# yuxng/PoseCNN

Measured on AMD Instinct MI355X. Metric: RGB-D frames/sec (640x480, 21 classes), higher is better.
Workload: dtype f32

## Files before the change

posecnn_amd/csrc/mfma_ring.h:

```cpp
#pragma once

namespace pcnn {

typedef float v4f __attribute__((ext_vector_type(4)));

__device__ __forceinline__ void glds16_s(const char* sbase, unsigned voff, unsigned lds_addr)
{
  asm volatile("s_mov_b32 m0, %2\n\tglobal_load_lds_dwordx4 %0, %1"
               :: "v"(voff), "s"(sbase), "s"(lds_addr) : "memory", "m0");
}

__device__ __forceinline__ int ring_src_col(int lr, int row) { return (lr ^ (row & 15)) * 4; }
__device__ __forceinline__ unsigned ring_chunk_bytes(int j, int lk, int lr) { return (unsigned)(((4 * j + lk) ^ lr) * 16); }

}

#define RING_DSREAD_B128(DST, ADDR, OFF) asm volatile("ds_read_b128 %0, %1 offset:%2" : "=v"(DST) : "v"(ADDR), "i"(OFF))

#define RING_GLOAD_B128(DST, SBASE, VOFF, OFF) \
  asm volatile("global_load_dwordx4 %0, %1, %2 offset:%3" : "=v"(DST) : "v"(VOFF), "s"(SBASE), "i"(OFF) : "memory")
```

posecnn_amd/csrc/wino_mfma.hip:

```cpp
#include <cstdlib>

#include "pcnn_device.h"
#include "mfma_ring.h"
#include "../../include/posecnn_hip_wino_packed.h"

namespace {

using namespace pcnn;

constexpr int WM_BC = 64;
constexpr int WM_KC = 64;
constexpr int WM_LD = 64;
constexpr int WM_NBUF = 3;
constexpr int WM_BT = 32;
constexpr int WM_NW = 4;
constexpr int WM_UB = WM_BC / 4 / WM_NW;

enum : int {
  ABL_NO_BARRIER = 1,
  ABL_NO_DMA = 2,
  ABL_NO_LDS_READS = 4,
  ABL_NO_MFMA = 8,
  ABL_NO_FOLD = 16,
  ABL_NO_EPILOGUE = 32,
  ABL_L2_OPERANDS = 64,
  ABL_NO_STORES = 128,
  ABL_EPI_REGS_ONLY = 256,
  ABL_NT_STORES = 512,
  ABL_NO_B_LOADS = 1024,
};

template <int POOL, int BSRC = 0, int ABL = 0, int ODD = 0>
__global__ __launch_bounds__(64 * WM_NW, 2) void wino43_mfma_kernel(
    const float* __restrict__ v, const float* __restrict__ ut, const float* __restrict__ bias,
    float* __restrict__ y, float* __restrict__ ypool, int H, int W, int Cin, int Cout, int Ht, int Wt,
    long long T, long long tiles_per_group, int relu, int nbt, int ncb, int ksplit, long long ysplit_stride, int mode)
{
  constexpr int RING = WM_NBUF * (WM_BT + (BSRC == 0 ? 64 : 0)) * WM_LD, STAGE2 = 2 * WM_BT * 4 * 64;
  __shared__ __attribute__((aligned(16))) float smem[RING > STAGE2 ? RING : STAGE2];

  const int x = blockIdx.x & 7, q = blockIdx.x >> 3;
  const bool cbmajor = (mode & 1) != 0;
  const int cb = cbmajor ? x : q % ncb;
  const int tb = cbmajor ? q : (q / ncb) * 8 + x;
  if (tb >= nbt) return;
  const int tb_data = (ABL & ABL_L2_OPERANDS) ? 0 : tb, cb_data = (ABL & ABL_L2_OPERANDS) ? 0 : cb;
  y += (long long)blockIdx.y * ysplit_stride;

  const int tid = threadIdx.x, lane = tid & 63;
  const int wave = __builtin_amdgcn_readfirstlane(tid >> 6);
  const int lr = lane & 15, lk = lane >> 4;
  const int nbg = (int)((tiles_per_group + WM_BT - 1) / WM_BT);
  const int grp = tb / nbg;
  const long long t0 = (long long)grp * tiles_per_group + (long long)(tb_data - (ABL & ABL_L2_OPERANDS ? 0 : grp * nbg)) * WM_BT;
  const long long tend = (long long)(grp + 1) * tiles_per_group;
  const float* utg = ut + (size_t)grp * 36 * Cout * Cin;
  const int ks = blockIdx.y;
  const int NK = Cin / WM_KC / ksplit;

  const int dr0 = 8 * wave + lk, dr1 = dr0 + 4;
  const int dc0 = ring_src_col(lr, dr0), dc1 = ring_src_col(lr, dr1);
  const int ur0 = 4 * WM_UB * wave + lk;
  const long long tlast = tend - 1;
  const long long ta0 = t0 + dr0 < tend ? t0 + dr0 : tlast, ta1 = t0 + dr1 < tend ? t0 + dr1 : tlast;
  const unsigned va0 = (unsigned)((ta0 * Cin + dc0) * 4), va1 = (unsigned)((ta1 * Cin + dc1) * 4);
  unsigned ub[WM_UB];
#pragma unroll
  for (int i = 0; i < WM_UB; i++) ub[i] = (unsigned)((((size_t)(cb_data * WM_BC + ur0 + 4 * i)) * Cin + ring_src_col(lr, ur0 + 4 * i)) * 4);
  const char* vbase = reinterpret_cast<const char*>(v);
  const char* ubase = reinterpret_cast<const char*>(utg);
  const long long vplane = T * Cin;
  const long long uplane = (long long)Cout * Cin;
  const int ldsw = 8 * wave * WM_LD;
  const int ldsu = 4 * WM_UB * wave * WM_LD;
  const unsigned lds_base_ = (unsigned)(unsigned long long)(__attribute__((address_space(3))) float*)smem;
  const unsigned lds_a0 = lds_base_ + (unsigned)ldsw * 4u;
  const unsigned lds_b0 = lds_base_ + (unsigned)(WM_NBUF * WM_BT * WM_LD + ldsu) * 4u;

  const float bv = bias ? bias[(size_t)grp * Cout + cb * WM_BC + 16 * wave + lr] : 0.f;
  v4f acc[6][2];
#pragma unroll
  for (int i = 0; i < 6; i++) acc[i][0] = acc[i][1] = (v4f){0.f, 0.f, 0.f, 0.f};
  typedef float v2f __attribute__((ext_vector_type(2)));
  v2f yo2[2][2][16];
#define YO(B_, I_, O_) yo2[B_][(I_) >> 1][O_][(I_) & 1]
#pragma unroll
  for (int b = 0; b < 2; b++)
#pragma unroll
    for (int i = 0; i < 2; i++)
#pragma unroll
      for (int o = 0; o < 16; o++) yo2[b][i][o] = (v2f){0.f, 0.f};

#define WM_DMA(BUF, VO, UO)                                                  \
  if constexpr (!(ABL & ABL_NO_DMA)) {                                       \
    const char* vs_ = vbase + (VO) * 4;                                      \
    const char* us_ = ubase + (UO) * 4;                                      \
    const unsigned la_ = lds_a0 + (unsigned)(BUF) * (WM_BT * WM_LD * 4);       \
    const unsigned lb_ = lds_b0 + (unsigned)(BUF) * (64 * WM_LD * 4);          \
    glds16_s(vs_, va0, la_);                                                 \
    glds16_s(vs_, va1, la_ + 4 * WM_LD * 4);                                 \
    if constexpr (BSRC == 0) {                                               \
      _Pragma("unroll") for (int i_ = 0; i_ < WM_UB; i_++)                    \
        glds16_s(us_, ub[i_], lb_ + 4 * i_ * WM_LD * 4);                      \
    }                                                                        \
  }

  int pnu = 0, pxi = 0, pkc = 0;
  constexpr int WM_USTEP = BSRC == 0 ? WM_KC : 16 * WM_KC;
  long long pvo = (long long)ks * NK * WM_KC;
  long long puo = BSRC == 0 ? pvo : ((long long)(cb_data * (WM_BC / 16) + wave) * (Cin / WM_KC) + (long long)ks * NK) * WM_USTEP;
  const long long kback = (long long)(NK - 1) * WM_KC, ukback = (long long)(NK - 1) * WM_USTEP;
  const long long dvx = 6 * vplane - kback, dux = 6 * uplane - ukback;
  const long long dvn = -29 * vplane - kback, dun = -29 * uplane - ukback;
#define WM_PF_ADVANCE()                                                                          \
  do {                                                                                           \
    if (pkc + 1 < NK) { pkc++; pvo += WM_KC; puo += WM_USTEP; }                 \
    else if (pxi < 5) { pkc = 0; pxi++; pvo += dvx; puo += dux; }        \
    else if (pnu < 5) { pkc = 0; pxi = 0; pnu++; pvo += dvn; puo += dun; }        \
  } while (0)
  v4f bq[4][2];
  if constexpr (BSRC == 1 && (ABL & ABL_NO_B_LOADS)) {
#pragma unroll
    for (int i = 0; i < 4; i++) bq[i][0] = bq[i][1] = (v4f){1.f, 1.f, 1.f, 1.f};
  }
  const unsigned vbo = 16u * (unsigned)lane;
  long long pub = 0;
#define WM_BLOAD(S, UO, J0)                                                  \
  if constexpr (!(ABL & ABL_NO_B_LOADS)) {                                   \
    const char* us_ = ubase + (UO) * 4;                                      \
    RING_GLOAD_B128(S[0], us_, vbo, (J0) * 1024);                            \
    RING_GLOAD_B128(S[1], us_, vbo, (J0) * 1024 + 1024);                     \
  }
  if constexpr (BSRC == 0) {
    { WM_DMA(0, pvo, puo); WM_PF_ADVANCE(); }
    { WM_DMA(1, pvo, puo); WM_PF_ADVANCE(); }
  } else {
    WM_BLOAD(bq[0], puo, 0);
    WM_BLOAD(bq[1], puo, 2);
    { WM_DMA(0, pvo, puo); WM_PF_ADVANCE(); }
    { WM_DMA(1, pvo, puo); pub = puo; WM_PF_ADVANCE(); }
  }
  int cur = 0;

  const int ra0 = lr * WM_LD, rb = (16 * wave + lr) * WM_LD;

  v4f xa0[2], xa1[2], xb[2], ya0[2], ya1[2], yb[2];
  const unsigned lds0 = (unsigned)(unsigned long long)(__attribute__((address_space(3))) float*)smem;
  unsigned adA[4], adB[4];
#pragma unroll
  for (int j = 0; j < 4; j++) {
    const unsigned chb = ring_chunk_bytes(j, lk, lr);
    adA[j] = lds0 + (unsigned)ra0 * 4u + chb;
    adB[j] = lds0 + (unsigned)(WM_NBUF * WM_BT * WM_LD + rb) * 4u + chb;
  }
#define WM_DSREAD(DST, ADDR, OFF)                                                                     \
  if constexpr (!(ABL & ABL_NO_LDS_READS)) RING_DSREAD_B128(DST, ADDR, OFF);                          \
  else asm volatile("" : "+v"(DST) : "v"(ADDR))
#define WM_READ_AT(SA0, SA1, SB, G0, CUR)                                                             \
  _Pragma("unroll") for (int g_ = 0; g_ < 2; g_++) {                                                  \
    WM_DSREAD(SB[g_], adB[(G0) + g_], (CUR) * (64 * WM_LD * 4));                                      \
    WM_DSREAD(SA0[g_], adA[(G0) + g_], (CUR) * (WM_BT * WM_LD * 4));                                  \
    WM_DSREAD(SA1[g_], adA[(G0) + g_], (CUR) * (WM_BT * WM_LD * 4) + 4096);       \
  }
#define WM_READ(SA0, SA1, SB, G0)                                                                     \
  if constexpr (ABL & ABL_NO_LDS_READS) { WM_READ_AT(SA0, SA1, SB, G0, 0); }    \
  else if (cur == 0) { WM_READ_AT(SA0, SA1, SB, G0, 0); }                                             \
  else if (cur == 1) { WM_READ_AT(SA0, SA1, SB, G0, 1); }                                             \
  else { WM_READ_AT(SA0, SA1, SB, G0, 2); }
#define WM_READA_AT(SA0, SA1, G0, CUR)                                                                \
  _Pragma("unroll") for (int g_ = 0; g_ < 2; g_++) {                                                  \
    WM_DSREAD(SA0[g_], adA[(G0) + g_], (CUR) * (WM_BT * WM_LD * 4));                                  \
    WM_DSREAD(SA1[g_], adA[(G0) + g_], (CUR) * (WM_BT * WM_LD * 4) + 4096);                           \
  }
#define WM_READA(SA0, SA1, G0)                                                                        \
  if constexpr (ABL & ABL_NO_LDS_READS) { WM_READA_AT(SA0, SA1, G0, 0); }                             \
  else if (cur == 0) { WM_READA_AT(SA0, SA1, G0, 0); }                                                \
  else if (cur == 1) { WM_READA_AT(SA0, SA1, G0, 1); }                                                \
  else { WM_READA_AT(SA0, SA1, G0, 2); }
  static_assert(WM_NBUF == 3, "WM_READ dispatches over a ring of three buffers");
#define WM_MFMA1(SA0, SA1, SB, G, ACC)                                                                \
  if constexpr (ABL & ABL_NO_MFMA) { asm volatile("" :: "v"(SA0[G]), "v"(SA1[G]), "v"(SB[G])); } else \
  _Pragma("unroll") for (int i_ = 0; i_ < 4; i_++) {                                                  \
    ACC[0] = __builtin_amdgcn_mfma_f32_16x16x4f32(SA0[G][i_], SB[G][i_], ACC[0], 0, 0, 0);            \
    ACC[1] = __builtin_amdgcn_mfma_f32_16x16x4f32(SA1[G][i_], SB[G][i_], ACC[1], 0, 0, 0);            \
  }
#define WM_MFMA(SA0, SA1, SB, ACC)                                                                    \
  WM_MFMA1(SA0, SA1, SB, 0, ACC) WM_MFMA1(SA0, SA1, SB, 1, ACC)
#define WM_MFMA1_Z(SA0, SA1, SB, G, ACC)                                                              \
  if constexpr (ABL & ABL_NO_MFMA) { asm volatile("" :: "v"(SA0[G]), "v"(SA1[G]), "v"(SB[G])); } else { \
    const v4f z_ = (v4f){0.f, 0.f, 0.f, 0.f};                                                         \
    ACC[0] = __builtin_amdgcn_mfma_f32_16x16x4f32(SA0[G][0], SB[G][0], z_, 0, 0, 0);                  \
    ACC[1] = __builtin_amdgcn_mfma_f32_16x16x4f32(SA1[G][0], SB[G][0], z_, 0, 0, 0);                  \
    _Pragma("unroll") for (int i_ = 1; i_ < 4; i_++) {                                                \
      ACC[0] = __builtin_amdgcn_mfma_f32_16x16x4f32(SA0[G][i_], SB[G][i_], ACC[0], 0, 0, 0);          \
      ACC[1] = __builtin_amdgcn_mfma_f32_16x16x4f32(SA1[G][i_], SB[G][i_], ACC[1], 0, 0, 0);          \
    }                                                                                                 \
  }
#define WM_FOLD(NU)                                                                                   \
  if constexpr (!(ABL & ABL_NO_FOLD)) {                                                               \
    const int n_ = (NU);                                                                              \
    const float c0 = n_ == 5 ? 0.f : 1.f;                                                             \
    const float c1 = n_ == 1 ? 1.f : n_ == 2 ? -1.f : n_ == 3 ? 2.f : n_ == 4 ? -2.f : 0.f;           \
    const float c2 = (n_ == 1 || n_ == 2) ? 1.f : (n_ == 3 || n_ == 4) ? 4.f : 0.f;                   \
    const float c3 = n_ == 1 ? 1.f : n_ == 2 ? -1.f : n_ == 3 ? 8.f : n_ == 4 ? -8.f : n_ == 5 ? 1.f : 0.f; \
     \
     \
     \
     \
     \
    _Pragma("unroll") for (int b_ = 0; b_ < 2; b_++)                                                \
      _Pragma("unroll") for (int h_ = 0; h_ < 2; h_++) {                                            \
        v2f m_[6], t_[4];                                                                           \
        _Pragma("unroll") for (int x_ = 0; x_ < 6; x_++) m_[x_] = (v2f){acc[x_][b_][2 * h_], acc[x_][b_][2 * h_ + 1]}; \
        const v2f s_ = m_[1] + m_[2], d_ = m_[1] - m_[2], S_ = m_[3] + m_[4], D_ = m_[3] - m_[4];   \
        t_[0] = (m_[0] + s_) + S_;                                                                  \
        t_[1] = __builtin_elementwise_fma((v2f){2.f, 2.f}, D_, d_);                                 \
        t_[2] = __builtin_elementwise_fma((v2f){4.f, 4.f}, S_, s_);                                 \
        t_[3] = __builtin_elementwise_fma((v2f){8.f, 8.f}, D_, d_) + m_[5];                         \
        _Pragma("unroll") for (int a_ = 0; a_ < 4; a_++) {                                          \
          yo2[b_][h_][4 * a_ + 0] = __builtin_elementwise_fma(t_[a_], (v2f){c0, c0}, yo2[b_][h_][4 * a_ + 0]); \
          yo2[b_][h_][4 * a_ + 1] = __builtin_elementwise_fma(t_[a_], (v2f){c1, c1}, yo2[b_][h_][4 * a_ + 1]); \
          yo2[b_][h_][4 * a_ + 2] = __builtin_elementwise_fma(t_[a_], (v2f){c2, c2}, yo2[b_][h_][4 * a_ + 2]); \
          yo2[b_][h_][4 * a_ + 3] = __builtin_elementwise_fma(t_[a_], (v2f){c3, c3}, yo2[b_][h_][4 * a_ + 3]); \
        }                                                                                           \
      }                                                                                             \
  }

#define WM_STAGE0(XI, XP)                                                                             \
  do {                                                                                                \
    if constexpr (ABL & ABL_NO_BARRIER) asm volatile("s_waitcnt vmcnt(4) lgkmcnt(0)" ::: "memory");   \
    else asm volatile("s_waitcnt vmcnt(6) lgkmcnt(0)\n\ts_barrier" ::: "memory");                     \
    WM_READ(xa0, xa1, xb, 0);                                                                         \
    __builtin_amdgcn_sched_barrier(0);    \
    if (kc > 0) { WM_MFMA(ya0, ya1, yb, acc[XI]); }                                                   \
    else if ((XI) > 0) { WM_MFMA(ya0, ya1, yb, acc[XP]); }                                            \
    else if (nu > 0) { WM_MFMA(ya0, ya1, yb, acc[5]); WM_FOLD(nup); }                                 \
    {                                                                                                 \
      const int nb = cur >= 1 ? cur - 1 : 2;            \
      WM_DMA(nb, pvo, puo);                                                                           \
      WM_PF_ADVANCE();                                                                                \
    }                                                                                                 \
    __builtin_amdgcn_sched_barrier(0);                                                                \
    asm volatile("s_waitcnt lgkmcnt(0)" ::: "memory");           \
    __builtin_amdgcn_sched_barrier(0);                                                                \
    if (kc == 0) { WM_MFMA1_Z(xa0, xa1, xb, 0, acc[XI]); }           \
    else { WM_MFMA1(xa0, xa1, xb, 0, acc[XI]); }                                                      \
    __builtin_amdgcn_sched_barrier(0);    \
    WM_READ(ya0, ya1, yb, 2);                                                                         \
    __builtin_amdgcn_sched_barrier(0);                                                                \
    WM_MFMA1(xa0, xa1, xb, 1, acc[XI]);                                                               \
    __builtin_amdgcn_sched_barrier(0);                                                                \
    asm volatile("s_waitcnt lgkmcnt(0)" ::: "memory");    \
    cur = cur == 2 ? 0 : cur + 1;                                                                     \
  } while (0)
  static_assert(2 + WM_UB == 6, "the stage barrier's vmcnt(6) counts the 2 + WM_UB DMA instructions a wave issues per stage");

  constexpr int WM_VM1 = WM_BT / 4 / WM_NW;
#define WM_YMFMA_R(SB, ACC)                                                                           \
  __builtin_amdgcn_sched_barrier(0); WM_MFMA(ya0, ya1, SB, ACC); __builtin_amdgcn_sched_barrier(0)
#define WM_STAGE1(XI, XP, P, KC)                                                                      \
  do {                                                                                                \
    if constexpr (ABL & ABL_NO_BARRIER) asm volatile("s_waitcnt vmcnt(2) lgkmcnt(0)" ::: "memory");   \
    else asm volatile("s_waitcnt vmcnt(2) lgkmcnt(0)\n\ts_barrier" ::: "memory");                     \
    WM_READA(xa0, xa1, 0);                                                                            \
    WM_BLOAD(bq[2 - 2 * (P)], pub, 0);                     \
    __builtin_amdgcn_sched_barrier(0);                                                                \
    if ((KC) > 0) { WM_YMFMA_R(bq[3 - 2 * (P)], acc[XI]); }                                           \
    else if ((XI) > 0) { WM_YMFMA_R(bq[3 - 2 * (P)], acc[XP]); }                                      \
    else if (nu > 0) { WM_YMFMA_R(bq[3 - 2 * (P)], acc[5]); WM_FOLD(nup); }                           \
    __builtin_amdgcn_sched_barrier(0);                                                                \
               \
    WM_BLOAD(bq[3 - 2 * (P)], pub, 2);                                                                \
    {                                                                                                 \
      const int nb = cur >= 1 ? cur - 1 : 2;            \
      WM_DMA(nb, pvo, puo);                                                                           \
      pub = puo;                                                                                      \
      WM_PF_ADVANCE();                                                                                \
    }                                                                                                 \
    __builtin_amdgcn_sched_barrier(0);                                                                \
    asm volatile("s_waitcnt lgkmcnt(0)" ::: "memory");           \
    __builtin_amdgcn_sched_barrier(0);                                                                \
    if ((KC) == 0) { WM_MFMA1_Z(xa0, xa1, bq[2 * (P)], 0, acc[XI]); }    \
    else { WM_MFMA1(xa0, xa1, bq[2 * (P)], 0, acc[XI]); }                                             \
    __builtin_amdgcn_sched_barrier(0);                                                                \
    WM_READA(ya0, ya1, 2);                                                                            \
    __builtin_amdgcn_sched_barrier(0);                                                                \
    WM_MFMA1(xa0, xa1, bq[2 * (P)], 1, acc[XI]);                                                      \
    __builtin_amdgcn_sched_barrier(0);                                                                \
    asm volatile("s_waitcnt lgkmcnt(0)" ::: "memory");                                                \
    cur = cur == 2 ? 0 : cur + 1;                                                                     \
  } while (0)
  static_assert(WM_VM1 == 2, "the stage barrier's vmcnt(2) of BSRC = 1 counts the A DMA instructions a wave issues per stage");
#define WM_PLANE_E(XI, XP) for (int kc = 0; kc < NK; kc += 2) { WM_STAGE1(XI, XP, 0, kc); WM_STAGE1(XI, XP, 1, kc + 1); }
#define WM_PLANE_O(XI, XP, P0)                                                                        \
  WM_STAGE1(XI, XP, P0, 0);                                                                           \
  for (int kc = 1; kc < NK; kc += 2) { WM_STAGE1(XI, XP, 1 - (P0), kc); WM_STAGE1(XI, XP, P0, kc + 1); }

  int nup = -1;
  if constexpr (BSRC == 0) {
    for (int nu = 0; nu < 6; nu++) {
      for (int kc = 0; kc < NK; kc++) WM_STAGE0(0, 5);
      for (int kc = 0; kc < NK; kc++) WM_STAGE0(1, 0);
      for (int kc = 0; kc < NK; kc++) WM_STAGE0(2, 1);
      for (int kc = 0; kc < NK; kc++) WM_STAGE0(3, 2);
      for (int kc = 0; kc < NK; kc++) WM_STAGE0(4, 3);
      for (int kc = 0; kc < NK; kc++) WM_STAGE0(5, 4);
      nup = nu;
    }
  } else if constexpr (ODD == 0) {
    for (int nu = 0; nu < 6; nu++) {
      WM_PLANE_E(0, 5) WM_PLANE_E(1, 0) WM_PLANE_E(2, 1) WM_PLANE_E(3, 2) WM_PLANE_E(4, 3) WM_PLANE_E(5, 4)
      nup = nu;
    }
  } else {
    for (int nu = 0; nu < 6; nu++) {
      WM_PLANE_O(0, 5, 0) WM_PLANE_O(1, 0, 1) WM_PLANE_O(2, 1, 0) WM_PLANE_O(3, 2, 1) WM_PLANE_O(4, 3, 0) WM_PLANE_O(5, 4, 1)
      nup = nu;
    }
  }
  if constexpr (BSRC == 0) {
    asm volatile("s_waitcnt lgkmcnt(0)" ::: "memory");
    __builtin_amdgcn_sched_barrier(0);
    WM_MFMA(ya0, ya1, yb, acc[5]);
  } else {
    asm volatile("s_waitcnt vmcnt(2) lgkmcnt(0)" ::: "memory");
    __builtin_amdgcn_sched_barrier(0);
    WM_MFMA(ya0, ya1, bq[3], acc[5]);
  }
  WM_FOLD(5);
  asm volatile("s_waitcnt vmcnt(0)" ::: "memory");
  __syncthreads();
#undef WM_STAGE0
#undef WM_STAGE1
#undef WM_YMFMA_R
#undef WM_PLANE_E
#undef WM_PLANE_O
#undef WM_BLOAD
#undef WM_READA
#undef WM_READA_AT
#undef WM_READ
#undef WM_READ_AT
#undef WM_DSREAD
#undef WM_MFMA
#undef WM_MFMA1
#undef WM_MFMA1_Z
#undef WM_FOLD
#undef WM_DMA
#undef WM_PF_ADVANCE

  if constexpr (ABL & ABL_EPI_REGS_ONLY) {
    const float bv_ = bv;
    float k_ = 0.f;
#pragma unroll
    for (int b = 0; b < 2; b++)
#pragma unroll
      for (int i = 0; i < 4; i++)
#pragma unroll
        for (int o = 0; o < 16; o++) { float val = YO(b, i, o) + bv_; if (relu) val = val > 0.f ? val : 0.f; k_ += val; }
    if (k_ == 12345.678f) y[tid] = k_;
    return;
  }
  if constexpr (ABL & ABL_NO_EPILOGUE) {
    float k_ = 0.f;
#pragma unroll
    for (int b = 0; b < 2; b++)
#pragma unroll
      for (int i = 0; i < 4; i++)
#pragma unroll
        for (int o = 0; o < 16; o++) k_ += YO(b, i, o);
#pragma unroll
    for (int x_ = 0; x_ < 6; x_++) k_ += acc[x_][0][0] + acc[x_][1][1];
    if (k_ == 12345.678f) y[tid] = k_;
    return;
  }
  const int col = 16 * wave + lr;
#pragma unroll
  for (int b = 0; b < 2; b++)
#pragma unroll
    for (int i = 0; i < 4; i++)
#pragma unroll
      for (int o = 0; o < 16; o++) {
        float val = YO(b, i, o) + bv;
        if (relu) val = val > 0.f ? val : 0.f;
        YO(b, i, o) = val;
      }

  constexpr int SYF = WM_BT * 4 * 64;
  const int wcol = col ^ (16 * lk);
  const int HtWt = Ht * Wt;
  const int bimg0 = (int)(t0 / HtWt);
  const int rem0 = (int)(t0 - (long long)bimg0 * HtWt);
  const int ty0 = rem0 / Wt, tx0 = rem0 - ty0 * Wt;
  const int re = (tid >> 4) & 3, rc4 = (tid & 15) * 4;
  int s_img[8], s_tyx[8];
#pragma unroll
  for (int r = 0; r < 8; r++) {
    const int tl = wave + WM_NW * r;
    const unsigned n = (unsigned)(tx0 + tl), q = n / (unsigned)Wt, tx = n - q * (unsigned)Wt;
    const unsigned m = (unsigned)ty0 + q, q2 = m / (unsigned)Ht, ty = m - q2 * (unsigned)Ht;
    s_img[r] = bimg0 + (int)q2;
    s_tyx[r] = t0 + tl < tend ? (int)(ty | (tx << 16)) : 0xffff;
  }
  if (POOL != 1) {
#pragma unroll
    for (int a = 0; a < 4; a++) {
      float* sY = smem + (a & 1) * SYF;
#pragma unroll
      for (int b = 0; b < 2; b++)
#pragma unroll
        for (int i = 0; i < 4; i++) {
          const int tl = 16 * b + 4 * lk + i;
#pragma unroll
          for (int e = 0; e < 4; e++) sY[(tl * 4 + e) * 64 + wcol] = YO(b, i, 4 * a + e);
        }
      __syncthreads();
#pragma unroll
      for (int r = 0; r < 8; r++) {
        const int tl = wave + WM_NW * r;
        const int ty = s_tyx[r] & 0xffff, tx = s_tyx[r] >> 16;
        const int oy = 4 * ty + a, ox = 4 * tx + re;
        if (oy < H && ox < W) {
          const v4f o4 = *reinterpret_cast<const v4f*>(&sY[(tl * 4 + re) * 64 + (rc4 ^ (16 * ((tl >> 2) & 3)))]);
          if constexpr (ABL & ABL_NO_STORES) { if (o4[0] == 12345.678f) y[tid] = o4[1]; }
          else if constexpr (ABL & ABL_NT_STORES) __builtin_nontemporal_store(o4, reinterpret_cast<v4f*>(y + (((long long)s_img[r] * H + oy) * W + ox) * Cout + cb * WM_BC + rc4));
          else *reinterpret_cast<v4f*>(y + (((long long)s_img[r] * H + oy) * W + ox) * Cout + cb * WM_BC + rc4) = o4;
        }
      }
    }
  }
  if (POOL != 0) {
    float* yp = POOL == 1 ? y : ypool;
    float* sY = smem;
    const int Hp = H / 2, Wp = W / 2;
#pragma unroll
    for (int b = 0; b < 2; b++)
#pragma unroll
      for (int i = 0; i < 4; i++) {
        const int tl = 16 * b + 4 * lk + i;
#pragma unroll
        for (int a2 = 0; a2 < 2; a2++)
#pragma unroll
          for (int e2 = 0; e2 < 2; e2++) {
            float p = YO(b, i, 4 * (2 * a2) + 2 * e2);
            const float p1 = YO(b, i, 4 * (2 * a2) + 2 * e2 + 1), p2 = YO(b, i, 4 * (2 * a2 + 1) + 2 * e2),
                        p3 = YO(b, i, 4 * (2 * a2 + 1) + 2 * e2 + 1);
            p = p1 > p ? p1 : p;
            p = p2 > p ? p2 : p;
            p = p3 > p ? p3 : p;
            sY[(tl * 4 + 2 * a2 + e2) * 64 + wcol] = p;
          }
      }
    __syncthreads();
#pragma unroll
    for (int r = 0; r < 8; r++) {
      const int tl = wave + WM_NW * r;
      const int ty = s_tyx[r] & 0xffff, tx = s_tyx[r] >> 16;
      const int py = 2 * ty + (re >> 1), px = 2 * tx + (re & 1);
      if (py < Hp && px < Wp)
        *reinterpret_cast<v4f*>(yp + (((long long)s_img[r] * Hp + py) * Wp + px) * Cout + cb * WM_BC + rc4) =
            *reinterpret_cast<const v4f*>(&sY[(tl * 4 + re) * 64 + (rc4 ^ (16 * ((tl >> 2) & 3)))]);
    }
  }
}

#undef YO

template <int POOL>
__global__ __launch_bounds__(256) void wino43_splitk_reduce_kernel(
    const float* __restrict__ part, int S, long long stride, const float* __restrict__ bias, int relu,
    float* __restrict__ y, float* __restrict__ ypool, int B, int H, int W, int C, int imgs_per_group)
{
  const int c4n = C >> 2;
  const int Ho = POOL ? H / 2 : H, Wo = POOL ? W / 2 : W;
  const long long total = (long long)B * Ho * Wo * c4n;
  for (long long i = (long long)blockIdx.x * 256 + threadIdx.x; i < total; i += (long long)gridDim.x * 256) {
    const int c4 = (int)(i % c4n) * 4;
    long long r = i / c4n;
    const int ox = (int)(r % Wo); r /= Wo;
    const int oy = (int)(r % Ho);
    const int b = (int)(r / Ho);
    const v4f bv = *reinterpret_cast<const v4f*>(bias + (size_t)(b / imgs_per_group) * C + c4);
    v4f best = (v4f){0.f, 0.f, 0.f, 0.f};
#pragma unroll
    for (int q = 0; q < (POOL ? 4 : 1); q++) {
      const int yy = POOL ? 2 * oy + (q >> 1) : oy, xx = POOL ? 2 * ox + (q & 1) : ox;
      const long long o = (((long long)b * H + yy) * W + xx) * C + c4;
      v4f v = *reinterpret_cast<const v4f*>(part + o);
      for (int s2 = 1; s2 < S; s2++) v += *reinterpret_cast<const v4f*>(part + s2 * stride + o);
      v += bv;
      if (relu) {
#pragma unroll
        for (int e = 0; e < 4; e++) v[e] = v[e] > 0.f ? v[e] : 0.f;
      }
      if (POOL != 1) *reinterpret_cast<v4f*>(y + o) = v;
      if (q == 0) best = v;
      else {
#pragma unroll
        for (int e = 0; e < 4; e++) best[e] = v[e] > best[e] ? v[e] : best[e];
      }
    }
    if (POOL != 0) {
      float* yp = POOL == 1 ? y : ypool;
      *reinterpret_cast<v4f*>(yp + (((long long)b * Ho + oy) * Wo + ox) * C + c4) = best;
    }
  }
}

int wino43_cin_split(long long nbt, int ncb, int Cin)
{
  const int NK = Cin / WM_KC;
  int S = 1;
  if (nbt * ncb >= 128) return 1;
  while (S < 8 && nbt * ncb * S * 2 <= 512 && NK % (2 * S) == 0) S *= 2;
  return S;
}

}

extern "C" int pcnn_winograd43_conv_workspace_bytes(int B, int H, int W, int Cin, int Cout, int groups, size_t* bytes)
{
  PCNN_REQUIRE(bytes, PCNN_ENULL, "winograd43_conv_workspace_bytes: NULL output");
  PCNN_REQUIRE(B >= 1 && H >= 1 && W >= 1 && Cin >= 64 && Cout >= 64 && groups >= 1 && B % groups == 0, PCNN_EINVAL,
               "winograd43_conv_workspace_bytes: bad shape");
  const long long tpg = (long long)B * ((H + 3) / 4) * ((W + 3) / 4) / groups;
  const int S = wino43_cin_split((long long)groups * ((tpg + WM_BT - 1) / WM_BT), Cout / WM_BC, Cin);
  *bytes = S > 1 ? sizeof(float) * ((size_t)S * B * H * W * Cout + (size_t)groups * Cout) : 0;
  return PCNN_OK;
}

static int wino43_conv_launch(bool packed, const float* v, const float* ut, const float* bias, int B, int H,
                              int W, int Cin, int Cout, int groups, int relu, int pool,
                              float* y, float* y_pool, void* workspace, size_t workspace_bytes,
                              void* stream_)
{
  PCNN_REQUIRE(B >= 1 && H >= 1 && W >= 1, PCNN_EINVAL, "winograd43_conv: bad shape %dx%dx%d", B, H, W);
  PCNN_REQUIRE(Cin >= 64 && Cin % 64 == 0, PCNN_EINVAL, "winograd43_conv: input channels must be a multiple of 64 (got %d)", Cin);
  PCNN_REQUIRE(Cout >= 64 && Cout % 64 == 0, PCNN_EINVAL, "winograd43_conv: output channels must be a multiple of 64 (got %d)", Cout);
  PCNN_REQUIRE(pool >= 0 && pool <= 2, PCNN_EINVAL, "winograd43_conv: pool must be 0 (none), 1 (pooled only) or 2 (both)");
  PCNN_REQUIRE(!pool || (H % 2 == 0 && W % 2 == 0), PCNN_EINVAL, "winograd43_conv: pooling needs even height/width");
  PCNN_REQUIRE(groups >= 1 && B % groups == 0, PCNN_EINVAL, "winograd43_conv: batch %d is not a multiple of groups %d", B, groups);
  PCNN_REQUIRE(v && ut && bias && y && (pool != 2 || y_pool), PCNN_ENULL, "winograd43_conv: NULL pointer");
  PCNN_REQUIRE(aligned16(v) && aligned16(ut) && aligned16(bias) && aligned16(y) && (pool != 2 || aligned16(y_pool)), PCNN_EINVAL,
               "winograd43_conv: pointers (v, ut, bias, y, y_pool) must be 16-byte aligned");
  hipStream_t stream = (hipStream_t)stream_;
  const int Ht = (H + 3) / 4, Wt = (W + 3) / 4;
  const long long T = (long long)B * Ht * Wt;
  const long long tpg = T / groups;
  const int ncb = Cout / WM_BC;
  const long long nbt = (long long)groups * ((tpg + WM_BT - 1) / WM_BT);
  const long long blocks = ((nbt + 7) / 8) * 8 * ncb;
  PCNN_REQUIRE(blocks < (1ll << 31), PCNN_EINVAL, "winograd43_conv: grid too large");
  PCNN_REQUIRE(T * Cin < (1ll << 30) && (long long)Cout * Cin < (1ll << 30), PCNN_EINVAL,
               "winograd43_conv: a transform plane of %lld x %d (or %d x %d) floats exceeds the kernel's 32-bit byte offsets", T, Cin, Cout, Cin);
  int S = wino43_cin_split(nbt, ncb, Cin);
  const size_t out_elems = (size_t)B * H * W * Cout;
  if (S > 1 && !(workspace && aligned16(workspace) && workspace_bytes >= sizeof(float) * (S * out_elems + (size_t)groups * Cout))) S = 1;
  static const int env_mode = [] { const char* e = getenv("PCNN_WINO_MODE"); return e ? atoi(e) : -1; }();
  const double u_bytes = 36.0 * Cout * (double)Cin * 4.0 * groups, v_bytes = 36.0 * (double)T * Cin * 4.0;
  int mode = (ncb == 8 && u_bytes > v_bytes) ? 1 : 0;
  if (env_mode >= 0) mode = ((env_mode & 1) && ncb == 8) ? 1 : 0;
  const long long nblocks = (mode & 1) ? 8 * nbt : blocks;
#define WM_GO_(K, Y, BIAS, RELU, KS, STRIDE) PCNN_LAUNCH(K, dim3((unsigned)nblocks, KS), dim3(64 * WM_NW), 0, stream, v, ut, BIAS, Y, y_pool, \
                             H, W, Cin, Cout, Ht, Wt, T, tpg, RELU, (int)nbt, ncb, KS, (long long)(STRIDE), mode)
#define WM_GO(P, Y, BIAS, RELU, KS, STRIDE)                                      \
  do {                                                                           \
    if (packed && ((Cin / WM_KC / (KS)) & 1)) WM_GO_((wino43_mfma_kernel<P, 1, 0, 1>), Y, BIAS, RELU, KS, STRIDE); \
    else if (packed) WM_GO_((wino43_mfma_kernel<P, 1>), Y, BIAS, RELU, KS, STRIDE);   \
    else WM_GO_((wino43_mfma_kernel<P>), Y, BIAS, RELU, KS, STRIDE);             \
  } while (0)
  if (S == 1) {
    if (pool == 0) WM_GO(0, y, bias, relu, 1, 0); else if (pool == 1) WM_GO(1, y, bias, relu, 1, 0); else WM_GO(2, y, bias, relu, 1, 0);
  } else {
    float* part = static_cast<float*>(workspace);
    WM_GO(0, part, (const float*)nullptr, 0, S, out_elems);
    const long long items = (long long)B * (pool ? (H / 2) * (W / 2) : H * W) * (Cout / 4);
    const unsigned rgrid = (unsigned)((items + 255) / 256 < 65536 ? (items + 255) / 256 : 65536);
    if (pool == 0)
      PCNN_LAUNCH(wino43_splitk_reduce_kernel<0>, dim3(rgrid), dim3(256), 0, stream, part, S, (long long)out_elems, bias, relu, y, y_pool, B, H, W, Cout, B / groups);
    else if (pool == 1)
      PCNN_LAUNCH(wino43_splitk_reduce_kernel<1>, dim3(rgrid), dim3(256), 0, stream, part, S, (long long)out_elems, bias, relu, y, y_pool, B, H, W, Cout, B / groups);
    else
      PCNN_LAUNCH(wino43_splitk_reduce_kernel<2>, dim3(rgrid), dim3(256), 0, stream, part, S, (long long)out_elems, bias, relu, y, y_pool, B, H, W, Cout, B / groups);
  }
  return check_launch(packed ? "winograd43_conv_packed_fwd" : "winograd43_conv_fwd");
}

extern "C" int pcnn_winograd43_conv_fwd(const float* v, const float* ut, const float* bias, int B, int H,
                                        int W, int Cin, int Cout, int groups, int relu, int pool,
                                        float* y, float* y_pool, void* workspace, size_t workspace_bytes,
                                        void* stream_)
{
  return wino43_conv_launch(false, v, ut, bias, B, H, W, Cin, Cout, groups, relu, pool, y, y_pool, workspace, workspace_bytes, stream_);
}

extern "C" int pcnn_winograd43_conv_packed_fwd(const float* v, const float* utp, const float* bias, int B, int H,
                                               int W, int Cin, int Cout, int groups, int relu, int pool,
                                               float* y, float* y_pool, void* workspace, size_t workspace_bytes,
                                               void* stream_)
{
  return wino43_conv_launch(true, v, utp, bias, B, H, W, Cin, Cout, groups, relu, pool, y, y_pool, workspace, workspace_bytes, stream_);
}

namespace {

__global__ __launch_bounds__(256) void wino43_pack_filters_kernel(const float* __restrict__ ut, float* __restrict__ utp,
                                                                  int Cin, int Cout, long long total4)
{
  const int nkc = Cin / WM_KC, n16n = Cout / 16;
  for (long long o = (long long)blockIdx.x * 256 + threadIdx.x; o < total4; o += (long long)gridDim.x * 256) {
    const int l = (int)(o & 63), j = (int)((o >> 6) & 3);
    long long r = o >> 8;
    const int kc = (int)(r % nkc); r /= nkc;
    const int n16 = (int)(r % n16n);
    const long long gk = r / n16n;
    const int lr = l & 15, lk = l >> 4;
    const long long src = (gk * Cout + 16 * n16 + lr) * Cin + 64 * kc + 16 * j + 4 * lk;
    *reinterpret_cast<v4f*>(utp + 4 * o) = *reinterpret_cast<const v4f*>(ut + src);
  }
}

}

extern "C" int pcnn_winograd43_pack_filters_fwd(const float* ut, int Cin, int Cout, int groups, float* utp, void* stream_)
{
  PCNN_REQUIRE(Cin >= 64 && Cin % 64 == 0, PCNN_EINVAL, "winograd43_pack_filters: input channels must be a multiple of 64 (got %d)", Cin);
  PCNN_REQUIRE(Cout >= 64 && Cout % 64 == 0, PCNN_EINVAL, "winograd43_pack_filters: output channels must be a multiple of 64 (got %d)", Cout);
  PCNN_REQUIRE(groups >= 1, PCNN_EINVAL, "winograd43_pack_filters: groups must be positive (got %d)", groups);
  PCNN_REQUIRE(ut && utp, PCNN_ENULL, "winograd43_pack_filters: NULL pointer");
  PCNN_REQUIRE(ut != utp, PCNN_EINVAL, "winograd43_pack_filters: not an in-place permutation");
  PCNN_REQUIRE(aligned16(ut) && aligned16(utp), PCNN_EINVAL, "winograd43_pack_filters: pointers (ut, utp) must be 16-byte aligned");
  hipStream_t stream = (hipStream_t)stream_;
  const long long total4 = (long long)groups * 36 * Cout * Cin / 4;
  const unsigned grid = (unsigned)((total4 + 255) / 256 < 65536 ? (total4 + 255) / 256 : 65536);
  PCNN_LAUNCH(wino43_pack_filters_kernel, dim3(grid), dim3(256), 0, stream, ut, utp, Cin, Cout, total4);
  return check_launch("winograd43_pack_filters_fwd");
}
```

Before: 840.4.

## Restructure Winograd epilogue with scalar store bases and fused bias-relu per row

Measured after the change: 840.2. About the same (-0.0%).

```diff
diff --git a/posecnn_amd/csrc/mfma_ring.h b/posecnn_amd/csrc/mfma_ring.h
--- a/posecnn_amd/csrc/mfma_ring.h
+++ b/posecnn_amd/csrc/mfma_ring.h
@@ -19,3 +19,10 @@
 
 #define RING_GLOAD_B128(DST, SBASE, VOFF, OFF) \
   asm volatile("global_load_dwordx4 %0, %1, %2 offset:%3" : "=v"(DST) : "v"(VOFF), "s"(SBASE), "i"(OFF) : "memory")
+
+#define RING_GSTORE_B128(SBASE, VOFF, DATA, MOD)                                                      \
+  do {                                                                                                \
+    unsigned long long sb_;                                                                           \
+    asm volatile("s_mov_b64 %0, %3\n\tglobal_store_dwordx4 %1, %2, %0" MOD "\n\ts_nop 1"             \
+                 : "=&s"(sb_) : "v"(VOFF), "v"(DATA), "s"(SBASE) : "memory");                         \
+  } while (0)
diff --git a/posecnn_amd/csrc/wino_mfma.hip b/posecnn_amd/csrc/wino_mfma.hip
--- a/posecnn_amd/csrc/wino_mfma.hip
+++ b/posecnn_amd/csrc/wino_mfma.hip
@@ -373,70 +373,109 @@
     if (k_ == 12345.678f) y[tid] = k_;
     return;
   }
-  const int col = 16 * wave + lr;
-#pragma unroll
-  for (int b = 0; b < 2; b++)
-#pragma unroll
-    for (int i = 0; i < 4; i++)
-#pragma unroll
-      for (int o = 0; o < 16; o++) {
-        float val = YO(b, i, o) + bv;
-        if (relu) val = val > 0.f ? val : 0.f;
-        YO(b, i, o) = val;
-      }
+  const int elane = (int)__builtin_amdgcn_mbcnt_hi(~0u, __builtin_amdgcn_mbcnt_lo(~0u, 0u));
+  const int elr = elane & 15, elk = elane >> 4;
+  const int col = 16 * wave + elr;
+#define WM_BIAS_RELU(B0, B1, I0, I1, O0, O1)                                                           \
+  if (relu) {                                                                                          \
+    _Pragma("unroll") for (int b_ = (B0); b_ < (B1); b_++)                                             \
+      _Pragma("unroll") for (int i_ = (I0); i_ < (I1); i_++)                                           \
+        _Pragma("unroll") for (int o_ = (O0); o_ < (O1); o_++) {                                       \
+          const float val = YO(b_, i_, o_) + bv;                                                       \
+          YO(b_, i_, o_) = val > 0.f ? val : 0.f;                                                      \
+        }                                                                                              \
+  } else {                                                                                             \
+    _Pragma("unroll") for (int b_ = (B0); b_ < (B1); b_++)                                             \
+      _Pragma("unroll") for (int i_ = (I0); i_ < (I1); i_++)                                           \
+        _Pragma("unroll") for (int o_ = (O0); o_ < (O1); o_++) YO(b_, i_, o_) = YO(b_, i_, o_) + bv;   \
+  }
 
   constexpr int SYF = WM_BT * 4 * 64;
-  const int wcol = col ^ (16 * lk);
-  const int HtWt = Ht * Wt;
-  const int bimg0 = (int)(t0 / HtWt);
-  const int rem0 = (int)(t0 - (long long)bimg0 * HtWt);
-  const int ty0 = rem0 / Wt, tx0 = rem0 - ty0 * Wt;
-  const int re = (tid >> 4) & 3, rc4 = (tid & 15) * 4;
-  int s_img[8], s_tyx[8];
-#pragma unroll
-  for (int r = 0; r < 8; r++) {
-    const int tl = wave + WM_NW * r;
-    const unsigned n = (unsigned)(tx0 + tl), q = n / (unsigned)Wt, tx = n - q * (unsigned)Wt;
-    const unsigned m = (unsigned)ty0 + q, q2 = m / (unsigned)Ht, ty = m - q2 * (unsigned)Ht;
-    s_img[r] = bimg0 + (int)q2;
-    s_tyx[r] = t0 + tl < tend ? (int)(ty | (tx << 16)) : 0xffff;
-  }
+  const int wcol = col ^ (16 * elk);
+  const int re = elk, rc4 = elr * 4;
+#define WM_SLOT_COORDS(LANE)                                                                           \
+  const unsigned HtWt = (unsigned)Ht * (unsigned)Wt;                                                   \
+  const unsigned l_t = (unsigned)t0 + (unsigned)(wave + WM_NW * ((LANE) & 7));                         \
+  const unsigned l_img = l_t / HtWt, l_rem = l_t - l_img * HtWt;                                       \
+  const unsigned l_ty = l_rem / (unsigned)Wt, l_tx = l_rem - l_ty * (unsigned)Wt;                      \
+  const bool l_live = (long long)l_t < tend
+#define WM_SLOT32(V, R) __builtin_amdgcn_readlane((int)(V), R)
+#define WM_SLOT64(V, R) (((unsigned long long)(unsigned)__builtin_amdgcn_readlane((int)((unsigned long long)(V) >> 32), R) << 32) | \
+                         (unsigned)__builtin_amdgcn_readlane((int)(unsigned)(unsigned long long)(V), R))
+  typedef __attribute__((address_space(3))) const float* lds_cfp;
+  lds_cfp srd[4];
+#pragma unroll
+  for (int c = 0; c < 4; c++) srd[c] = (lds_cfp)smem + (wave * 4 + re) * 64 + (rc4 ^ (16 * c));
+#define WM_EPI_READ(O4, BUF)                                                                           \
+  _Pragma("unroll") for (int r = 0; r < 8; r++)                                                        \
+    O4[r] = *reinterpret_cast<__attribute__((address_space(3))) const v4f*>(srd[r & 3] + (BUF) * SYF + r * (WM_NW * 4 * 64)); \
+  asm volatile("" ::: "memory")
   if (POOL != 1) {
+    WM_SLOT_COORDS(elane);
+    const int l_rows = l_live ? min(H - 4 * (int)l_ty, 4) : 0, l_cols = min(W - 4 * (int)l_tx, 4);
+    const unsigned long long l_base = (unsigned long long)y + 4ull * (unsigned long long)((((long long)l_img * H + 4 * l_ty) * W + 4 * l_tx) * Cout + cb * WM_BC);
+    const int l_whole = l_cols == 4 ? l_rows : 0;
+    const long long pitch = 4ll * W * Cout;
+    const unsigned vst = (unsigned)(re * Cout + rc4) * 4u;
+    int s_rc[8];
+    unsigned long long s_base[8];
+#pragma unroll
+    for (int r = 0; r < 8; r++) { s_rc[r] = WM_SLOT32(l_rows | (l_cols << 4), r); s_base[r] = WM_SLOT64(l_base, r); }
 #pragma unroll
     for (int a = 0; a < 4; a++) {
       float* sY = smem + (a & 1) * SYF;
+      WM_BIAS_RELU(0, 2, 0, 4, 4 * a, 4 * a + 4);
 #pragma unroll
       for (int b = 0; b < 2; b++)
 #pragma unroll
         for (int i = 0; i < 4; i++) {
-          const int tl = 16 * b + 4 * lk + i;
+          const int tl = 16 * b + 4 * elk + i;
 #pragma unroll
           for (int e = 0; e < 4; e++) sY[(tl * 4 + e) * 64 + wcol] = YO(b, i, 4 * a + e);
         }
       __syncthreads();
-#pragma unroll
-      for (int r = 0; r < 8; r++) {
-        const int tl = wave + WM_NW * r;
-        const int ty = s_tyx[r] & 0xffff, tx = s_tyx[r] >> 16;
-        const int oy = 4 * ty + a, ox = 4 * tx + re;
-        if (oy < H && ox < W) {
-          const v4f o4 = *reinterpret_cast<const v4f*>(&sY[(tl * 4 + re) * 64 + (rc4 ^ (16 * ((tl >> 2) & 3)))]);
-          if constexpr (ABL & ABL_NO_STORES) { if (o4[0] == 12345.678f) y[tid] = o4[1]; }
-          else if constexpr (ABL & ABL_NT_STORES) __builtin_nontemporal_store(o4, reinterpret_cast<v4f*>(y + (((long long)s_img[r] * H + oy) * W + ox) * Cout + cb * WM_BC + rc4));
-          else *reinterpret_cast<v4f*>(y + (((long long)s_img[r] * H + oy) * W + ox) * Cout + cb * WM_BC + rc4) = o4;
+      v4f o4[8];
+      WM_EPI_READ(o4, a & 1);
+      const unsigned long long arow = (unsigned long long)(a * pitch);
+#define WM_EPI_STORE(R)                                                                                \
+      do {                                                                                             \
+        const char* dst = reinterpret_cast<const char*>(s_base[R] + arow);    \
+        if constexpr (ABL & ABL_NO_STORES) { if (o4[R][0] == 12345.678f) y[tid] = o4[R][1]; }          \
+        else if constexpr (ABL & ABL_NT_STORES) RING_GSTORE_B128(dst, vst, o4[R], " nt");              \
+        else RING_GSTORE_B128(dst, vst, o4[R], "");                                                    \
+      } while (0)
+      if ((__builtin_amdgcn_ballot_w64(a < l_whole) & 0xffull) == 0xffull) {
+#pragma unroll
+        for (int r = 0; r < 8; r++) WM_EPI_STORE(r);
+      } else {
+#pragma unroll
+        for (int r = 0; r < 8; r++) {
+          const int rows = s_rc[r] & 15, cols = s_rc[r] >> 4;
+          if (a < rows) {
+            if (cols == 4) WM_EPI_STORE(r);
+            else if (re < cols) WM_EPI_STORE(r);
+          }
         }
       }
+#undef WM_EPI_STORE
     }
   }
   if (POOL != 0) {
     float* yp = POOL == 1 ? y : ypool;
     float* sY = smem;
     const int Hp = H / 2, Wp = W / 2;
+    int plane = elane;
+    if (POOL == 2) asm volatile("" : "+v"(plane));
+    WM_SLOT_COORDS(plane);
+    const int l_rows = l_live ? min(Hp - 2 * (int)l_ty, 2) : 0, l_cols = min(Wp - 2 * (int)l_tx, 2);
+    const unsigned long long l_base = (unsigned long long)yp + 4ull * (unsigned long long)((((long long)l_img * Hp + 2 * l_ty) * Wp + 2 * l_tx) * Cout + cb * WM_BC);
+    const unsigned vst = (unsigned)(((re >> 1) * Wp + (re & 1)) * Cout + rc4) * 4u;
 #pragma unroll
     for (int b = 0; b < 2; b++)
 #pragma unroll
       for (int i = 0; i < 4; i++) {
-        const int tl = 16 * b + 4 * lk + i;
+        const int tl = 16 * b + 4 * elk + i;
+        if (POOL == 1) { WM_BIAS_RELU(b, b + 1, i, i + 1, 0, 16); }
 #pragma unroll
         for (int a2 = 0; a2 < 2; a2++)
 #pragma unroll
@@ -451,16 +490,29 @@
           }
       }
     __syncthreads();
-#pragma unroll
-    for (int r = 0; r < 8; r++) {
-      const int tl = wave + WM_NW * r;
-      const int ty = s_tyx[r] & 0xffff, tx = s_tyx[r] >> 16;
-      const int py = 2 * ty + (re >> 1), px = 2 * tx + (re & 1);
-      if (py < Hp && px < Wp)
-        *reinterpret_cast<v4f*>(yp + (((long long)s_img[r] * Hp + py) * Wp + px) * Cout + cb * WM_BC + rc4) =
-            *reinterpret_cast<const v4f*>(&sY[(tl * 4 + re) * 64 + (rc4 ^ (16 * ((tl >> 2) & 3)))]);
+    v4f o4[8];
+    WM_EPI_READ(o4, 0);
+    if ((__builtin_amdgcn_ballot_w64(l_rows == 2 && l_cols == 2) & 0xffull) == 0xffull) {
+#pragma unroll
+      for (int r = 0; r < 8; r++) RING_GSTORE_B128(reinterpret_cast<const char*>(WM_SLOT64(l_base, r)), vst, o4[r], "");
+    } else {
+#pragma unroll
+      for (int r = 0; r < 8; r++) {
+        const int rc = WM_SLOT32(l_rows | (l_cols << 4), r);
+        const int rows = rc & 15, cols = rc >> 4;
+        if (rows > 0) {
+          const char* dst = reinterpret_cast<const char*>(WM_SLOT64(l_base, r));
+          if (rows == 2 && cols == 2) RING_GSTORE_B128(dst, vst, o4[r], "");
+          else if ((re >> 1) < rows && (re & 1) < cols) RING_GSTORE_B128(dst, vst, o4[r], "");
+        }
+      }
     }
   }
+#undef WM_BIAS_RELU
+#undef WM_SLOT_COORDS
+#undef WM_EPI_READ
+#undef WM_SLOT32
+#undef WM_SLOT64
 }
 
 #undef YO
```
